# PKU-VCL-Geometry/GeoSplatting

Hardware: AMD Instinct MI355X
Metric: fwd+bwd views/sec at 2M Gaussians, 800x800 (higher is better)
Workload: dtype f32

## Files before the change

geosplatting_amd/csrc/gs_raster.hip:

```cpp
#include "gs_common.h"
#include "gs_tone.h"
#include <stdlib.h>

#pragma clang fp contract(off)

#define GS_TILE 16
#define GS_ALPHA_MIN (1.0f / 255.0f)

#ifdef GS_RASTER_STATS
__device__ unsigned long long g_raster_stats[8];
extern "C" int gs_raster_stats_read(unsigned long long* host8, int reset)
{
    if (hipMemcpyFromSymbol(host8, HIP_SYMBOL(g_raster_stats), sizeof(unsigned long long) * 8) != hipSuccess) return -1;
    if (reset) { unsigned long long z[8] = {0}; if (hipMemcpyToSymbol(HIP_SYMBOL(g_raster_stats), z, sizeof(z)) != hipSuccess) return -1; }
    return 0;
}
__device__ unsigned long long g_raster_stats2[8];
extern "C" int gs_raster_stats2_read(unsigned long long* host8, int reset)
{
    if (hipMemcpyFromSymbol(host8, HIP_SYMBOL(g_raster_stats2), sizeof(unsigned long long) * 8) != hipSuccess) return -1;
    if (reset) { unsigned long long z[8] = {0}; if (hipMemcpyToSymbol(HIP_SYMBOL(g_raster_stats2), z, sizeof(z)) != hipSuccess) return -1; }
    return 0;
}
__device__ unsigned long long g_raster_stats3[8];
// ... 642 lines not shown
    int bin_final = -1;
    float v_rc[CD];
#pragma unroll
    for (int k = 0; k < CD; ++k) v_rc[k] = 0.0f;
    if (inside) {
        const size_t pid = (size_t)pyi * W + pxi;
        const float a_out = alphas[pid];
        T_final = 1.0f - a_out;
        bin_final = last_ids[pid];
        if (CD == 3 && tone.v_image) {
#pragma clang fp contract(off)
            const float e = tone.exposure[0];
            const float r = tone.render[3 * pid], gch = tone.render[3 * pid + 1], bl = tone.render[3 * pid + 2];
            const float4 g = tone.v_image[pid];
            const float gx = g.x * tone_grad(tone.mode, r * e), gy = g.y * tone_grad(tone.mode, gch * e), gz = g.z * tone_grad(tone.mode, bl * e);
            v_rc[0] = gx * e; v_rc[1] = gy * e; v_rc[2] = gz * e;
            v_a = tone.mode == GS_TONE_NONE ? g.w * e : g.w;
            v_exp = gx * r + gy * gch + gz * bl + (tone.mode == GS_TONE_NONE ? g.w * a_out : 0.0f);
        } else {
            v_a = v_alphas[pid];
#pragma unroll
            for (int k = 0; k < CD; ++k) if (k < D) v_rc[k] = v_render[pid * D + k];
        }
    }
    if (CD == 3 && tone.v_image) {
        v_exp = gs_wave_sum(v_exp);
        if (lane == 0 && v_exp != 0.0f) gs_atomic_add(tone.v_exposure, v_exp);
    }
    float bg_dot = 0.0f;
    if (background) {
#pragma unroll
        for (int k = 0; k < CD; ++k) if (k < D) bg_dot += background[k] * v_rc[k];
    }
    if (CD > 3) for (int k = 0; k < D; ++k) vrp[k * 64 + lane] = v_rc[k < CD ? k : 0];
    float T = T_final;
    float zacc = T_final * v_a - T_final * bg_dot;
    const unsigned long long lane_lt = (1ull << lane) - 1ull;

    int top = bin_final;
#pragma unroll
    for (int off = 32; off >= 1; off >>= 1) top = max(top, __shfl_xor(top, off, 64));
    if (top >= end) top = end - 1;

    int qhead = 0, qcount = 0;
    top = __builtin_amdgcn_readfirstlane(top);
    RawBatch raw0, raw1, raw2;
    raw_load(raw0, rec0, rec1, rec2, top - lane, top - lane >= start);
    raw_load(raw1, rec0, rec1, rec2, top - 64 - lane, top - 64 - lane >= start);
    raw_load(raw2, rec0, rec1, rec2, top - 128 - lane, top - 128 - lane >= start);
    int phase = 0;
    for (;;) {
        { GS_PHASE_BEGIN();
#define BWD_FILL_STEP(B)                                                                                               \
        {                                                                                                              \
            const unsigned long long act_b = __ballot(bin_final >= top - 63);                                          \
            int n_hit = 0;                                                                                             \
            raw_wait(B);                                                                                               \
            if (act_b != 0ull) {                                                                                       \
                float rcx, rcy, rex, rey;                                                                              \
                active_rect_c(act_b, qx0, qy0, rcx, rcy, rex, rey);                                                    \
                GS_STAT(4, 1);                                                                                         \
                n_hit = lanes_cull_append(q, B, top - lane >= start, top - lane, lane, rcx, rcy, rex, rey, qhead + qcount); \
            }                                                                                                          \
            raw_load(B, rec0, rec1, rec2, top - 192 - lane, top - 192 - lane >= start);                                \
            qcount += n_hit;                                                                                           \
            top -= 64;                                                                                                 \
        }
        LANES_FILL(qcount < 64 && top >= start, BWD_FILL_STEP)
#undef BWD_FILL_STEP
        GS_PHASE_END(0); }
        if (qcount == 0) break;
        int nb = qcount < 64 ? qcount : 64;
        lanes_lds_sync();
        GS_PHASE_BEGIN();
        const int idx_low = q.idx[(qhead + nb - 1) & (GS_LANES_Q - 1)];
        const bool live = bin_final >= idx_low;
        const unsigned long long act = __ballot(live);
        const int myslot = (qhead + lane) & (GS_LANES_Q - 1);
        const float4 ra4 = q.a[myslot];
        const float2 rb4 = q.b[myslot];
        unsigned long long pm = 0ull;
        if (act != 0ull) {
            int xmin, xmax, ymin, ymax;
            active_rect_i(act, xmin, xmax, ymin, ymax);
            pm = record_pixel_mask(lane < nb, ra4.x, ra4.y, ra4.z, ra4.w, rb4.x, rb4.y, qx0, qy0, xmin, xmax, ymin, ymax) & act;
        }
        const int cnt = __popcll(pm);
        int cum = cnt;
        cum = gs_wave_incl_scan(cum);
        if (__ballot(cum > GS_PAIR_CAP) != 0ull) {
            nb = min(nb, __popcll(__ballot(cum <= GS_PAIR_CAP)));
            if (lane >= nb) pm = 0ull;
        }
        msk[lane] = pm;
        pbase[lane] = cum - cnt;
        if (CD > 3) {
            const float* cg = colors + (size_t)__float_as_int(q.c[myslot].w) * D;
            for (int k = 0; k < D; ++k) colp[k * 64 + lane] = lane < nb ? cg[k] : 0.0f;
        }
        unsigned long long list = gs_bit_transpose64(pm, lane);
        GS_STAT(5, nb);
#ifdef GS_RASTER_STATS
        GS_STAT2(1, 1);
        GS_STAT2_ALL(0, __popcll(list));
        { int _mx = __popcll(list);
          for (int _o = 32; _o >= 1; _o >>= 1) _mx = max(_mx, __shfl_xor(_mx, _o, 64));
          GS_STAT2(6, _mx); }
#endif
        lanes_lds_sync();
        GS_PHASE_END(1);
        long long _pw0 = 0;
#ifdef GS_RASTER_PHASES
        if (blockIdx.x == 0 && threadIdx.x == 0) { _pw0 = (long long)__builtin_readcyclecounter(); atomicAdd(&g_raster_stats[6], 1ull); }
#endif
        while (__ballot(list != 0ull) != 0ull) {
            GS_STAT(6, 1);
#ifdef GS_RASTER_PHASES
            if (blockIdx.x == 0 && threadIdx.x == 0) atomicAdd(&g_raster_stats[5], 1ull);
#endif
            const bool has0 = list != 0ull;
            const int j0 = gs_pop_lowest(list);
            const bool has1 = list != 0ull;
            const int j1 = gs_pop_lowest(list);
            const int slot0 = (qhead + j0) & (GS_LANES_Q - 1), slot1 = (qhead + j1) & (GS_LANES_Q - 1);
            const float4 a0 = q.a[slot0], a1 = q.a[slot1];
            const float2 b0 = q.b[slot0], b1 = q.b[slot1];
            const float4 c0 = q.c[slot0], c1 = q.c[slot1];
            const int idx0 = q.idx[slot0], idx1 = q.idx[slot1];
            const int e0 = pbase[j0] + __popcll(msk[j0] & lane_lt), e1 = pbase[j1] + __popcll(msk[j1] & lane_lt);
            v2f sigma, ov, alpha, ra;
            {
#pragma clang fp contract(off)
                const v2f d0 = v2f{a0.x, a0.y} - pxy, d1 = v2f{a1.x, a1.y} - pxy;
                const v2f p0 = v2f{a0.z, a0.w} * v2f{d0.x, d0.x}, p1 = v2f{a1.z, a1.w} * v2f{d1.x, d1.x};
                sigma.x = gs_sigma_xy(d0, p0, b0.x);
                sigma.y = gs_sigma_xy(d1, p1, b1.x);
                ov = v2f{b0.y, b1.y} * gs_exp_neg_live2(sigma);
                alpha = __builtin_elementwise_min(ov, (v2f)(0.999f));
                ra = gs_rcp_exact2((v2f)(1.0f) - alpha);
            }
            const bool ok0 = has0 && idx0 <= bin_final && sigma.x >= 0.0f && alpha.x >= GS_ALPHA_MIN;
            const bool ok1 = has1 && idx1 <= bin_final && sigma.y >= 0.0f && alpha.y >= GS_ALPHA_MIN;
            {
                const float Tn = T * ra.x;
                const float fac = ok0 ? alpha.x * Tn : 0.0f;
                float cv;
                if (CD <= 3) {
                    cv = c0.x * v_rc[0];
                    if (CD > 1) cv = fmaf(c0.y, v_rc[1], cv);
                    if (CD > 2) cv = fmaf(c0.z, v_rc[2], cv);
                } else {
                    cv = 0.0f;
#pragma unroll
                    for (int k = 0; k < CD; ++k) if (k < D) cv = fmaf(colp[k * 64 + j0], v_rc[k], cv);
                }
                const float v_alpha = fmaf(Tn, cv, ra.x * zacc);
                const float s_out = (ok0 && ov.x <= 0.999f) ? -ov.x * v_alpha : 0.0f;
                zacc = fmaf(-fac, cv, zacc);
                T = ok0 ? Tn : T;
#ifdef GS_RASTER_STATS
                if (ok0) GS_STAT_ALL(7, 1);
                if (has0 && !ok0) { if (idx0 > bin_final) GS_STAT2_ALL(2, 1); else GS_STAT2_ALL(3, 1); }
#endif
                if (has0) pairbuf[e0] = make_float2(s_out, fac);
            }
            {
                const float Tn = T * ra.y;
                const float fac = ok1 ? alpha.y * Tn : 0.0f;
                float cv;
                if (CD <= 3) {
                    cv = c1.x * v_rc[0];
                    if (CD > 1) cv = fmaf(c1.y, v_rc[1], cv);
                    if (CD > 2) cv = fmaf(c1.z, v_rc[2], cv);
                } else {
                    cv = 0.0f;
#pragma unroll
                    for (int k = 0; k < CD; ++k) if (k < D) cv = fmaf(colp[k * 64 + j1], v_rc[k], cv);
                }
                const float v_alpha = fmaf(Tn, cv, ra.y * zacc);
                const float s_out = (ok1 && ov.y <= 0.999f) ? -ov.y * v_alpha : 0.0f;
                zacc = fmaf(-fac, cv, zacc);
                T = ok1 ? Tn : T;
#ifdef GS_RASTER_STATS
                if (ok1) GS_STAT_ALL(7, 1);
                if (has1 && !ok1) { if (idx1 > bin_final) GS_STAT2_ALL(2, 1); else GS_STAT2_ALL(3, 1); }
#endif
                if (has1) pairbuf[e1] = make_float2(s_out, fac);
            }
        }
        lanes_lds_sync();
#ifdef GS_RASTER_PHASES
        if (blockIdx.x == 0 && threadIdx.x == 0) { const long long _t = (long long)__builtin_readcyclecounter(); atomicAdd(&g_raster_stats[2], (unsigned long long)(_t - _pw0)); _pw0 = _t; }
#endif
        float sum[NV];
        {
            const float X = ra4.x - ((float)qx0 + 0.5f), Y = ra4.y - ((float)qy0 + 0.5f);
            unsigned long long m = pm;
            int e = cum - cnt;
            float m0 = 0.0f, mxy = 0.0f, c2 = 0.0f;
            v2f m1 = (v2f)(0.0f), m2 = (v2f)(0.0f), c01 = (v2f)(0.0f);
            float csum[CD > 3 ? CD : 1];
#pragma unroll
            for (int k = 0; k < (CD > 3 ? CD : 1); ++k) csum[k] = 0.0f;
            while (__ballot(m != 0ull) != 0ull) {
                GS_STAT2(7, 1);
#ifdef GS_RASTER_PHASES
                if (blockIdx.x == 0 && threadIdx.x == 0) atomicAdd(&g_raster_stats[7], 1ull);
#endif
                const bool has = m != 0ull;
                const int p = gs_pop_lowest(m);
                const float2 sfr = pairbuf[has ? e : 0];
                float4 vr = make_float4(0.f, 0.f, 0.f, 0.f);
                if (CD <= 3) { vr.x = __shfl(v_rc[0], p, 64); vr.y = CD > 1 ? __shfl(v_rc[1], p, 64) : 0.0f; vr.z = CD > 2 ? __shfl(v_rc[2], p, 64) : 0.0f; }
                if (CD > 3) {
                    const float fw = has ? sfr.y : 0.0f;
#pragma unroll
                    for (int k = 0; k < CD; ++k) if (k < D) csum[k] = fmaf(fw, vrp[k * 64 + p], csum[k]);
                }
                e += has ? 1 : 0;
                const float s_w = has ? sfr.x : 0.0f, f_w = has ? sfr.y : 0.0f;
                const v2f d = v2f{X, Y} - v2f{(float)(p & 7), (float)(p >> 3)};
                const v2f sd = d * s_w;
                m0 += s_w;
                m1 += sd;
                m2 = __builtin_elementwise_fma(sd, d, m2);
                mxy = fmaf(sd.x, d.y, mxy);
                c01 = __builtin_elementwise_fma((v2f)(f_w), v2f{vr.x, vr.y}, c01);
                if (CD > 2) c2 = fmaf(f_w, vr.z, c2);
            }
            sum[0] = m0; sum[1] = m1.x; sum[2] = m1.y; sum[3] = m2.x; sum[4] = mxy; sum[5] = m2.y;
            if (CD <= 3) {
                sum[6] = c01.x;
                if (CD > 1) sum[7] = c01.y;
                if (CD > 2) sum[8] = c2;
            } else {
#pragma unroll
                for (int k = 0; k < CD; ++k) sum[6 + k] = csum[k];
            }
        }
        lanes_lds_sync();
#ifdef GS_RASTER_PHASES
        if (blockIdx.x == 0 && threadIdx.x == 0) { const long long _t = (long long)__builtin_readcyclecounter(); atomicAdd(&g_raster_stats[3], (unsigned long long)(_t - _pw0)); _pw0 = _t; }
#endif
        {
            const float ga = ra4.z, gb = ra4.w, gc = rb4.x, go = rb4.y;
            const float M0 = sum[0], Mx = sum[1], My = sum[2];
            float out[NV];
            out[0] = (2.0f * ga) * Mx + gb * My;
            out[1] = gb * Mx + (2.0f * gc) * My;
            out[2] = 0.5f * sum[3]; out[3] = sum[4]; out[4] = 0.5f * sum[5];
            out[5] = (M0 != 0.0f) ? -M0 / go : 0.0f;
#pragma unroll
            for (int k = 0; k < CD; ++k) out[6 + k] = sum[6 + k];
            if (lane < nb) {
#pragma unroll
                for (int k = 0; k < NV; ++k) stage[lane * NV + k] = out[k];
            }
        }
        lanes_lds_sync();
        {
            const int r = lane / NV, k = lane - r * NV;
            for (int it = 0; it * RPI < nb; ++it) {
                const int j = it * RPI + r;
                if (r < RPI && j < nb && k < 6 + D) {
                    const float v = stage[j * NV + k];
                    if (v != 0.0f) {
                        const int g = __float_as_int(q.c[(qhead + j) & (GS_LANES_Q - 1)].w);
                        gs_atomic_add(v_packed + (size_t)g * rec_stride + k, v);
                    }
                }
            }
        }
        lanes_lds_sync();
#ifdef GS_RASTER_PHASES
        if (blockIdx.x == 0 && threadIdx.x == 0) atomicAdd(&g_raster_stats[4], (unsigned long long)((long long)__builtin_readcyclecounter() - _pw0));
#endif
        qhead = (qhead + nb) & (GS_LANES_Q - 1);
        qcount -= nb;
    }
    raw_drain(raw0, raw1, raw2);
    GS_TL_END();
}

static constexpr int GS_LOG_PAIR_CAP = 790;
#ifndef GS_LOG_ASSIST_MAX
#define GS_LOG_ASSIST_MAX 16
#endif
static_assert(GS_LOG_ASSIST_MAX >= 0 && GS_LOG_ASSIST_MAX <= 64, "an assisted trip serves at most the 64 pixels of one wave");
struct LogLds {
    static constexpr int Q_BYTES = 64 * (16 + 16 + 8 + 4);
    static constexpr int OFF_MSK = Q_BYTES;
    static constexpr int OFF_BASE = OFF_MSK + 64 * 8;
    static constexpr int OFF_PAIR = OFF_BASE + 64 * 4;
    static constexpr int OFF_APIX = OFF_PAIR + (GS_LOG_PAIR_CAP + 2) * 8;
    static constexpr int WAVE_BYTES = OFF_APIX + (GS_LOG_ASSIST_MAX > 16 ? GS_LOG_ASSIST_MAX : 16) * 4;
};

template <int CTRL>
__device__ __forceinline__ float gs_row_shr(float ident, float src)
{
    return __builtin_bit_cast(float, __builtin_amdgcn_update_dpp(__builtin_bit_cast(int, ident), __builtin_bit_cast(int, src), CTRL, 0xf, 0xf, false));
}

template <int CD>
__global__ void __launch_bounds__(256)
raster_bwd_log_kernel(int W, int H, int tile_w, int n_tiles, int D, const int32_t* __restrict__ tile_order,
                      const float4* __restrict__ rec0, const float4* __restrict__ rec1, const float4* __restrict__ rec2,
                      const float* __restrict__ background, GsCount ic, const int32_t* __restrict__ offsets,
                      const float* __restrict__ alphas, const int32_t* __restrict__ last_ids,
                      const float* __restrict__ v_render, const float* __restrict__ v_alphas,
                      float* __restrict__ v_packed, int rec_stride, ToneBwd tone, CullLog log, BwdOrder bo)
{
    const int n_isects = (int)gs_count(ic);
#if defined(GS_RASTER_STATS) && !defined(GS_RASTER_PHASES)
    int walk_hist[8] = { 0, 0, 0, 0, 0, 0, 0, 0 };
#endif
    static_assert(CD <= 3, "colours come from the record stream (D <= 3)");
    using LD = LogLds;
    constexpr int NV = 6 + CD;
    constexpr int RPI = 64 / NV;
    static_assert(64 * NV * 4 <= GS_LOG_PAIR_CAP * 8, "the commit staging aliases the pair buffer");
    extern __shared__ __align__(16) unsigned char gs_lds_raw[];
    const int lane = threadIdx.x & 63, wave = __builtin_amdgcn_readfirstlane((int)(threadIdx.x >> 6));
    int tile;
    if (bo.bcount) {
        const int c = bo.bcount[lane];
        int incl = c;
        incl = gs_wave_incl_scan(incl);
        const unsigned long long above = __ballot(incl > (int)blockIdx.x);
        const int b = above ? __builtin_ctzll(above) : 63;
        const int before = __builtin_amdgcn_readlane(incl - c, b);
        tile = __builtin_amdgcn_readlane(incl, 63) == n_tiles
                   ? __builtin_amdgcn_readfirstlane(bo.blist[(size_t)b * n_tiles + ((int)blockIdx.x - before)]) : tile_order[blockIdx.x];
    } else {
        tile = tile_order[blockIdx.x];
    }
    const int tx = tile % tile_w, ty = tile / tile_w;
    const int qx0 = tx * GS_TILE + (wave & 1) * 8, qy0 = ty * GS_TILE + (wave >> 1) * 8;
    const int pxi = qx0 + (lane & 7), pyi = qy0 + (lane >> 3);
    const bool inside = pxi < W && pyi < H;
    const float px = (float)pxi + 0.5f, py = (float)pyi + 0.5f;
    const v2f pxy = v2f{px, py};

    const int start = offsets[tile];
    const int end = (tile == n_tiles - 1) ? n_isects : offsets[tile + 1];
    GS_TL_BEGIN(end - start);
    if (end <= start) { GS_TL_END(); return; }

    unsigned char* wbase = gs_lds_raw + (size_t)wave * LD::WAVE_BYTES;
    float4* qa = (float4*)wbase; float4* qc = qa + 64; float2* qb = (float2*)(qc + 64); int* qidx = (int*)(qb + 64);
    unsigned long long* msk = (unsigned long long*)(wbase + LD::OFF_MSK);
    int* pbase = (int*)(wbase + LD::OFF_BASE);
    float2* pairbuf = (float2*)(wbase + LD::OFF_PAIR);
    int* apix = (int*)(wbase + LD::OFF_APIX);
    float* stage = (float*)(wbase + LD::OFF_PAIR);

    float T_final = 1.0f, v_a = 0.0f, v_exp = 0.0f;
    int bin_final = -1;
    float v_rc[CD];
#pragma unroll
    for (int k = 0; k < CD; ++k) v_rc[k] = 0.0f;
    if (inside) {
        const size_t pid = (size_t)pyi * W + pxi;
        const float a_out = alphas[pid];
        T_final = 1.0f - a_out;
        bin_final = last_ids[pid];
        if (CD == 3 && tone.v_image) {
#pragma clang fp contract(off)
            const float e = tone.exposure[0];
            const float r = tone.render[3 * pid], gch = tone.render[3 * pid + 1], bl = tone.render[3 * pid + 2];
            const float4 g = tone.v_image[pid];
            const float gx = g.x * tone_grad(tone.mode, r * e), gy = g.y * tone_grad(tone.mode, gch * e), gz = g.z * tone_grad(tone.mode, bl * e);
            v_rc[0] = gx * e; v_rc[1] = gy * e; v_rc[2] = gz * e;
            v_a = tone.mode == GS_TONE_NONE ? g.w * e : g.w;
            v_exp = gx * r + gy * gch + gz * bl + (tone.mode == GS_TONE_NONE ? g.w * a_out : 0.0f);
        } else {
            v_a = v_alphas[pid];
#pragma unroll
            for (int k = 0; k < CD; ++k) if (k < D) v_rc[k] = v_render[pid * D + k];
        }
    }
    if (CD == 3 && tone.v_image) {
        v_exp = gs_wave_sum(v_exp);
        if (lane == 0 && v_exp != 0.0f) gs_atomic_add(tone.v_exposure, v_exp);
    }
    float bg_dot = 0.0f;
    if (background) {
#pragma unroll
        for (int k = 0; k < CD; ++k) if (k < D) bg_dot += background[k] * v_rc[k];
    }
    float T = T_final;
    float zacc = T_final * v_a - T_final * bg_dot;
    const unsigned long long lane_lt = (1ull << lane) - 1ull;

    int pos = __builtin_amdgcn_readfirstlane(log.count[4 * tile + wave]);
    if (pos <= 0) { GS_TL_END(); return; }
    const size_t log_base = 4 * (size_t)start + (size_t)wave * (size_t)(end - start);
    const int32_t* lidx = log.idx + log_base;
    const unsigned long long* lmsk = log.mask + log_base;
    int e_idx, g_idx; unsigned long long e_msk, g_msk;
    float4 g0, g1, g2;
    {
        const int e = pos - 1 - lane;
        const int es = e >= 0 ? e : 0;
        g_idx = lidx[es]; g_msk = e >= 0 ? lmsk[es] : 0ull;
        g0 = rec0[g_idx]; g1 = rec1[g_idx]; g2 = rec2[g_idx];
        const int e2 = pos - 65 - lane;
        const int es2 = e2 >= 0 ? e2 : 0;
        e_idx = lidx[es2]; e_msk = e2 >= 0 ? lmsk[es2] : 0ull;
    }
    while (pos > 0) {
        const int nb = pos < 64 ? pos : 64;
        const float4 c0 = g0, c1 = g1, c2 = g2;
        const int c_idx = g_idx;
        const unsigned long long c_msk = g_msk;
        g_idx = e_idx; g_msk = e_msk;
        g0 = rec0[g_idx]; g1 = rec1[g_idx]; g2 = rec2[g_idx];
        {
            const int e2 = pos - 129 - lane;
            const int es2 = e2 >= 0 ? e2 : 0;
            e_idx = lidx[es2]; e_msk = e2 >= 0 ? lmsk[es2] : 0ull;
        }
        pos -= nb;
        GS_PHASE_BEGIN();
        lanes_lds_sync();
        qa[lane] = c0; qb[lane] = make_float2(c1.x, c1.y); qc[lane] = c2; qidx[lane] = c_idx;
        GS_STAT(5, nb);
        const int idx_low = __builtin_amdgcn_readlane(c_idx, nb - 1);
        const bool live = bin_final >= idx_low;
        const unsigned long long act = __ballot(live);
        const unsigned long long pm = lane < nb ? (c_msk & act) : 0ull;
        if (__ballot(pm != 0ull) == 0ull) { GS_PHASE_END(1); continue; }
        const float4 ra4 = c0;
        const float2 rb4 = make_float2(c1.x, c1.y);
        const int cnt = __popcll(pm);
        int cum = cnt;
        cum = gs_wave_incl_scan(cum);
        GS_PHASE_END(1);
        int r0 = 0, cumbase = 0;
        while (r0 < nb) {
            const int r1 = r0 + __popcll(__ballot(lane >= r0 && lane < nb && (cum - cumbase) <= GS_LOG_PAIR_CAP));
            const bool mine = lane >= r0 && lane < r1;
            const unsigned long long pms = mine ? pm : 0ull;
            lanes_lds_sync();
            msk[lane] = pms;
            pbase[lane] = cum - cnt - cumbase;
            unsigned long long list = gs_bit_transpose64(pms, lane);
#ifdef GS_RASTER_STATS
            GS_STAT2(1, 1);
            GS_STAT2_ALL(0, __popcll(list));
#endif
            lanes_lds_sync();
            long long _pw0 = 0;
#ifdef GS_RASTER_PHASES
            if (blockIdx.x == 0 && threadIdx.x == 0) { _pw0 = (long long)__builtin_readcyclecounter(); atomicAdd(&g_raster_stats[6], 1ull); }
#endif
            if (__ballot(list != 0ull) != 0ull) do {
                GS_STAT(6, 1);
#if defined(GS_RASTER_STATS) && !defined(GS_RASTER_PHASES)
                { const int na = __popcll(__ballot(list != 0ull));
#pragma unroll
                  for (int k = 0; k < 8; ++k) walk_hist[k] += (na > 8 * k && na <= 8 * k + 8) ? 1 : 0; }
#endif
#ifdef GS_RASTER_PHASES
                if (blockIdx.x == 0 && threadIdx.x == 0) atomicAdd(&g_raster_stats[5], 1ull);
#endif
#if GS_LOG_ASSIST_MAX > 0
                {
                    const unsigned long long am = __ballot(list != 0ull);
                    const int na = __popcll(am);
                    if (na <= GS_LOG_ASSIST_MAX && __ballot(__popcll(list) > 2) != 0ull) {
                        const int gs = na <= 8 ? 3 : (GS_LOG_ASSIST_MAX <= 16 || na <= 16) ? 2 : na <= 32 ? 1 : 0, G = 1 << gs;
                        const int rank = __popcll(am & lane_lt);
                        lanes_lds_sync();
                        if (list != 0ull) apix[rank] = lane;
                        lanes_lds_sync();
                        const int g = lane >> gs, h = lane & (G - 1);
                        const bool grp = g < na;
                        const int p = grp ? apix[g] : 0;
                        const int pa = p << 2;
                        unsigned long long L = ((unsigned long long)(unsigned)__builtin_amdgcn_ds_bpermute(pa, (int)(unsigned)(list >> 32)) << 32) |
                                               (unsigned long long)(unsigned)__builtin_amdgcn_ds_bpermute(pa, (int)(unsigned)list);
                        const float T0 = __builtin_bit_cast(float, __builtin_amdgcn_ds_bpermute(pa, __builtin_bit_cast(int, T)));
                        const float Z0 = __builtin_bit_cast(float, __builtin_amdgcn_ds_bpermute(pa, __builtin_bit_cast(int, zacc)));
                        const int bf = __builtin_amdgcn_ds_bpermute(pa, bin_final);
                        float vr[CD];
#pragma unroll
                        for (int c = 0; c < CD; ++c) vr[c] = __builtin_bit_cast(float, __builtin_amdgcn_ds_bpermute(pa, __builtin_bit_cast(int, v_rc[c])));
                        if (!grp) L = 0ull;
                        for (int i = 0; i < G - 1; ++i) L = (i < h) ? (L & (L - 1ull)) : L;
                        const bool has = L != 0ull;
                        const int j = gs_pop_lowest(L);
                        const float4 a = qa[j]; const float2 b = qb[j]; const float4 cc = qc[j];
                        const int idx = qidx[j];
                        const unsigned long long below = (1ull << p) - 1ull;
                        const int e = pbase[j] + __popcll(msk[j] & below);
                        float sigma, ov, alpha, ra;
                        {
#pragma clang fp contract(off)
                            const v2f d = v2f{a.x, a.y} - v2f{(float)(qx0 + (p & 7)) + 0.5f, (float)(qy0 + (p >> 3)) + 0.5f};
                            const v2f pp = v2f{a.z, a.w} * v2f{d.x, d.x};
                            sigma = gs_sigma_xy(d, pp, b.x);
                            ov = b.y * __builtin_amdgcn_exp2f(sigma * -1.4426950408889634f);
                            alpha = fminf(ov, 0.999f);
                            const float x = 1.0f - alpha;
                            const float r0 = __builtin_amdgcn_rcpf(x);
                            ra = fmaf(r0, fmaf(-x, r0, 1.0f), r0);
                        }
                        const bool ok = has & (idx <= bf) & (sigma >= 0.0f) & (alpha >= GS_ALPHA_MIN);
                        float cv = cc.x * vr[0];
                        if (CD > 1) cv = fmaf(cc.y, vr[1], cv);
                        if (CD > 2) cv = fmaf(cc.z, vr[2], cv);
                        float pi = ok ? ra : 1.0f;
                        { const float t = gs_row_shr<0x111>(1.0f, pi); pi *= (h >= 1) ? t : 1.0f; }
                        { const float t = gs_row_shr<0x112>(1.0f, pi); pi *= (h >= 2) ? t : 1.0f; }
                        { const float t = gs_row_shr<0x114>(1.0f, pi); pi *= (h >= 4) ? t : 1.0f; }
                        float pe = gs_row_shr<0x111>(1.0f, pi); pe = (h >= 1) ? pe : 1.0f;
                        const float Tb = T0 * pe, Tn = Tb * ra;
                        const float fac = ok ? alpha * Tn : 0.0f;
                        float si = fac * cv;
                        { const float t = gs_row_shr<0x111>(0.0f, si); si += (h >= 1) ? t : 0.0f; }
                        { const float t = gs_row_shr<0x112>(0.0f, si); si += (h >= 2) ? t : 0.0f; }
                        { const float t = gs_row_shr<0x114>(0.0f, si); si += (h >= 4) ? t : 0.0f; }
                        float se = gs_row_shr<0x111>(0.0f, si); se = (h >= 1) ? se : 0.0f;
                        const float zb = Z0 - se;
                        const float v_alpha = fmaf(Tn, cv, ra * zb);
                        const float s_out = (ok && ov <= 0.999f) ? -ov * v_alpha : 0.0f;
#ifdef GS_RASTER_STATS
                        if (ok) GS_STAT_ALL(7, 1);
                        if (has && !ok) { if (idx > bf) GS_STAT2_ALL(2, 1); else GS_STAT2_ALL(3, 1); }
#endif
                        pairbuf[has ? e : GS_LOG_PAIR_CAP] = make_float2(s_out, fac);
                        const float T_end = T0 * pi, Z_end = Z0 - si;
                        const int src = (((rank << gs) + G - 1) & 63) << 2;
                        const float Tg = __builtin_bit_cast(float, __builtin_amdgcn_ds_bpermute(src, __builtin_bit_cast(int, T_end)));
                        const float Zg = __builtin_bit_cast(float, __builtin_amdgcn_ds_bpermute(src, __builtin_bit_cast(int, Z_end)));
                        const unsigned Llo = (unsigned)__builtin_amdgcn_ds_bpermute(src, (int)(unsigned)L);
                        const unsigned Lhi = (unsigned)__builtin_amdgcn_ds_bpermute(src, (int)(unsigned)(L >> 32));
                        if (list != 0ull) { T = Tg; zacc = Zg; list = ((unsigned long long)Lhi << 32) | Llo; }
                        continue;
                    }
                }
#endif
                const bool has0 = list != 0ull;
                const int j0 = gs_pop_lowest(list);
                const bool has1 = list != 0ull;
                const int j1 = gs_pop_lowest(list);
                const float4 a0 = qa[j0], a1 = qa[j1];
                const float2 b0 = qb[j0], b1 = qb[j1];
                const float4 cc0 = qc[j0], cc1 = qc[j1];
                const int idx0 = qidx[j0], idx1 = qidx[j1];
                const int e0 = pbase[j0] + __popcll(msk[j0] & lane_lt), e1 = pbase[j1] + __popcll(msk[j1] & lane_lt);
                v2f sigma, ov, alpha, ra;
                {
#pragma clang fp contract(off)
                    const v2f d0 = v2f{a0.x, a0.y} - pxy, d1 = v2f{a1.x, a1.y} - pxy;
                    const v2f p0 = v2f{a0.z, a0.w} * v2f{d0.x, d0.x}, p1 = v2f{a1.z, a1.w} * v2f{d1.x, d1.x};
                    sigma.x = gs_sigma_xy(d0, p0, b0.x);
                    sigma.y = gs_sigma_xy(d1, p1, b1.x);
#ifndef GS_BWD_LOG_EXACT_MATH
                    ov = v2f{b0.y, b1.y} * v2f{__builtin_amdgcn_exp2f(sigma.x * -1.4426950408889634f), __builtin_amdgcn_exp2f(sigma.y * -1.4426950408889634f)};
                    alpha = __builtin_elementwise_min(ov, (v2f)(0.999f));
                    {
                        const v2f x = (v2f)(1.0f) - alpha;
                        const v2f r0 = v2f{__builtin_amdgcn_rcpf(x.x), __builtin_amdgcn_rcpf(x.y)};
                        ra = __builtin_elementwise_fma(r0, __builtin_elementwise_fma(-x, r0, (v2f)(1.0f)), r0);
                    }
#else
                    ov = v2f{b0.y, b1.y} * gs_exp_neg_live2(sigma);
                    alpha = __builtin_elementwise_min(ov, (v2f)(0.999f));
                    ra = gs_rcp_exact2((v2f)(1.0f) - alpha);
#endif
                }
                const bool ok0 = has0 & (idx0 <= bin_final) & (sigma.x >= 0.0f) & (alpha.x >= GS_ALPHA_MIN);
                const bool ok1 = has1 & (idx1 <= bin_final) & (sigma.y >= 0.0f) & (alpha.y >= GS_ALPHA_MIN);
                {
                    const float Tn = T * ra.x;
                    const float fac = ok0 ? alpha.x * Tn : 0.0f;
                    float cv = cc0.x * v_rc[0];
                    if (CD > 1) cv = fmaf(cc0.y, v_rc[1], cv);
                    if (CD > 2) cv = fmaf(cc0.z, v_rc[2], cv);
                    const float v_alpha = fmaf(Tn, cv, ra.x * zacc);
                    const float s_out = (ok0 && ov.x <= 0.999f) ? -ov.x * v_alpha : 0.0f;
                    zacc = fmaf(-fac, cv, zacc);
                    T = ok0 ? Tn : T;
#ifdef GS_RASTER_STATS
                    if (ok0) GS_STAT_ALL(7, 1);
                    if (has0 && !ok0) { if (idx0 > bin_final) GS_STAT2_ALL(2, 1); else GS_STAT2_ALL(3, 1); }
#endif
                    pairbuf[has0 ? e0 : GS_LOG_PAIR_CAP] = make_float2(s_out, fac);
                }
                {
                    const float Tn = T * ra.y;
                    const float fac = ok1 ? alpha.y * Tn : 0.0f;
                    float cv = cc1.x * v_rc[0];
                    if (CD > 1) cv = fmaf(cc1.y, v_rc[1], cv);
                    if (CD > 2) cv = fmaf(cc1.z, v_rc[2], cv);
                    const float v_alpha = fmaf(Tn, cv, ra.y * zacc);
                    const float s_out = (ok1 && ov.y <= 0.999f) ? -ov.y * v_alpha : 0.0f;
                    zacc = fmaf(-fac, cv, zacc);
                    T = ok1 ? Tn : T;
#ifdef GS_RASTER_STATS
                    if (ok1) GS_STAT_ALL(7, 1);
                    if (has1 && !ok1) { if (idx1 > bin_final) GS_STAT2_ALL(2, 1); else GS_STAT2_ALL(3, 1); }
#endif
                    pairbuf[has1 ? e1 : GS_LOG_PAIR_CAP] = make_float2(s_out, fac);
                }
            } while (__ballot(list != 0ull) != 0ull);
            lanes_lds_sync();
#ifdef GS_RASTER_PHASES
            if (blockIdx.x == 0 && threadIdx.x == 0) { const long long _t = (long long)__builtin_readcyclecounter(); atomicAdd(&g_raster_stats[2], (unsigned long long)(_t - _pw0)); _pw0 = _t; }
#endif
            float sum[NV];
            {
                const float X = ra4.x - ((float)qx0 + 0.5f), Y = ra4.y - ((float)qy0 + 0.5f);
                unsigned long long m = pms;
                int e = cum - cnt - cumbase;
                float m0 = 0.0f, mxy = 0.0f, c2s = 0.0f;
                v2f m1 = (v2f)(0.0f), m2 = (v2f)(0.0f), c01 = (v2f)(0.0f);
                if (__ballot(m != 0ull) != 0ull) do {
                    GS_STAT2(7, 1);
#ifdef GS_RASTER_PHASES
                    if (blockIdx.x == 0 && threadIdx.x == 0) atomicAdd(&g_raster_stats[7], 1ull);
#endif
                    const bool has = m != 0ull;
                    const int p = gs_pop_lowest(m);
                    const float2 sfr = pairbuf[has ? e : 0];
                    float4 vr;
                    vr.x = __shfl(v_rc[0], p, 64); vr.y = CD > 1 ? __shfl(v_rc[1], p, 64) : 0.0f; vr.z = CD > 2 ? __shfl(v_rc[2], p, 64) : 0.0f; vr.w = 0.0f;
                    e += has ? 1 : 0;
                    const float s_w = has ? sfr.x : 0.0f, f_w = has ? sfr.y : 0.0f;
                    const v2f d = v2f{X, Y} - v2f{(float)(p & 7), (float)(p >> 3)};
                    const v2f sd = d * s_w;
                    m0 += s_w;
                    m1 += sd;
                    m2 = __builtin_elementwise_fma(sd, d, m2);
                    mxy = fmaf(sd.x, d.y, mxy);
                    c01 = __builtin_elementwise_fma((v2f)(f_w), v2f{vr.x, vr.y}, c01);
                    if (CD > 2) c2s = fmaf(f_w, vr.z, c2s);
                } while (__ballot(m != 0ull) != 0ull);
                sum[0] = m0; sum[1] = m1.x; sum[2] = m1.y; sum[3] = m2.x; sum[4] = mxy; sum[5] = m2.y;
                sum[6] = c01.x;
                if (CD > 1) sum[7] = c01.y;
                if (CD > 2) sum[8] = c2s;
            }
            lanes_lds_sync();
#ifdef GS_RASTER_PHASES
            if (blockIdx.x == 0 && threadIdx.x == 0) { const long long _t = (long long)__builtin_readcyclecounter(); atomicAdd(&g_raster_stats[3], (unsigned long long)(_t - _pw0)); _pw0 = _t; }
#endif
            {
                const float ga = ra4.z, gb = ra4.w, gc = rb4.x, go = rb4.y;
                const float M0 = sum[0], Mx = sum[1], My = sum[2];
                float out[NV];
                out[0] = (2.0f * ga) * Mx + gb * My;
                out[1] = gb * Mx + (2.0f * gc) * My;
                out[2] = 0.5f * sum[3]; out[3] = sum[4]; out[4] = 0.5f * sum[5];
                out[5] = (M0 != 0.0f) ? -M0 / go : 0.0f;
#pragma unroll
                for (int k = 0; k < CD; ++k) out[6 + k] = sum[6 + k];
                if (mine) {
#pragma unroll
                    for (int k = 0; k < NV; ++k) stage[lane * NV + k] = out[k];
                }
            }
            lanes_lds_sync();
            {
                const int r = lane / NV, k = lane - r * NV;
                for (int it = 0; r0 + it * RPI < r1; ++it) {
                    const int j = r0 + it * RPI + r;
                    if (r < RPI && j < r1 && k < 6 + D) {
                        const float v = stage[j * NV + k];
                        if (v != 0.0f) {
                            const int g = __float_as_int(qc[j].w);
                            gs_atomic_add(v_packed + (size_t)g * rec_stride + k, v);
                        }
                    }
                }
            }
#ifdef GS_RASTER_PHASES
            if (blockIdx.x == 0 && threadIdx.x == 0) atomicAdd(&g_raster_stats[4], (unsigned long long)((long long)__builtin_readcyclecounter() - _pw0));
#endif
            cumbase = __builtin_amdgcn_readlane(cum, r1 - 1);
            r0 = r1;
        }
    }
#if defined(GS_RASTER_STATS) && !defined(GS_RASTER_PHASES)
    if (lane == 0) {
#pragma unroll
        for (int k = 0; k < 8; ++k) if (walk_hist[k]) atomicAdd(&g_raster_stats3[k], (unsigned long long)walk_hist[k]);
    }
#endif
    GS_TL_END();
}

#define GS_RASTER_BLOCKS_PER_CU 4
static int gs_raster_blocks_per_cu() { return GS_RASTER_BLOCKS_PER_CU; }
static size_t gs_raster_lds_pad() { return (size_t)(160 * 1024 / gs_raster_blocks_per_cu()) - 1024; }
static size_t gs_raster_lds(size_t natural)
{
    const size_t pad = gs_raster_lds_pad();
    if (natural >= pad) return natural;
    if ((size_t)(gs_raster_blocks_per_cu() + 1) * (natural + 512) > (size_t)160 * 1024) return natural;
    return pad;
}
static size_t align256(size_t x) { return (x + 255) & ~(size_t)255; }

extern "C" size_t gs_raster_ws_bytes(int64_t n_isects, int V, int W, int H, int tile_size)
{
    if (tile_size <= 0) return 0;
    const size_t tiles = (size_t)((W + tile_size - 1) / tile_size) * (size_t)((H + tile_size - 1) / tile_size);
    const size_t n = n_isects > 0 ? (size_t)n_isects : 1;
    const size_t v = V > 0 ? (size_t)V : 1;
    return 3 * align256(n * sizeof(float4)) + align256(tiles * sizeof(int32_t)) + align256(64 * sizeof(int32_t)) +
           align256(64 * tiles * sizeof(int32_t)) + align256(4 * v * sizeof(float4));
}

struct RasterWs {
    float4 *rec0, *rec1, *rec2;
    int32_t* order;
    BwdOrder bo;
    float4* vis;
};
static RasterWs carve(void* ws, int64_t n_isects, int V, int tiles)
{
    const size_t n = n_isects > 0 ? (size_t)n_isects : 1;
    const size_t v = V > 0 ? (size_t)V : 1;
    char* p = (char*)ws;
    RasterWs r;
    r.rec0 = (float4*)p; p += align256(n * sizeof(float4));
    r.rec1 = (float4*)p; p += align256(n * sizeof(float4));
    r.rec2 = (float4*)p; p += align256(n * sizeof(float4));
    r.order = (int32_t*)p; p += align256((size_t)tiles * sizeof(int32_t));
    r.bo.bcount = (int32_t*)p; p += align256(64 * sizeof(int32_t));
    r.bo.blist = (int32_t*)p; p += align256(64 * (size_t)tiles * sizeof(int32_t));
    r.vis = (float4*)p;
    return r;
}

struct RasterOpts {
    const int64_t* counts = nullptr;
    ToneFwd tone_fwd = { 0, nullptr, nullptr };
    ToneBwd tone_bwd = { 0, nullptr, nullptr, nullptr, nullptr };
    CullLog log = { nullptr, nullptr, nullptr };
};
static GsCount isect_count(int64_t n, const RasterOpts& o)
{
    return GsCount{ (long long)n, o.counts ? (const long long*)o.counts + 1 : nullptr };
}

template <int CD>
static int launch_fwd(int W, int H, int D, const RasterWs& ws, const float* colors, const float* background,
                      int64_t n_isects, const int32_t* offsets, float* render, float* alphas, int32_t* last_ids,
                      hipStream_t s, const RasterOpts& o)
{
    const int tile_w = (W + GS_TILE - 1) / GS_TILE, tile_h = (H + GS_TILE - 1) / GS_TILE;
    if (o.tone_fwd.image && !(CD == 3 && D == 3 && background == nullptr)) {
        gs_set_error("gs_raster_composite_tone: needs D == 3 and no background");
        return GS_EINVAL;
    }
    {
        const size_t planes = CD > 3 ? 4 * (size_t)2 * (size_t)D * 64 * sizeof(float) : 0;
        const size_t lds = gs_raster_lds(4 * (size_t)GS_WIN_Q_BYTES + planes);
        if (lds > 64 * 1024)
            GS_CHECK_HIP(hipFuncSetAttribute((const void*)raster_fwd_window_kernel<CD>, hipFuncAttributeMaxDynamicSharedMemorySize, (int)lds));
        hipLaunchKernelGGL(raster_fwd_window_kernel<CD>, dim3(tile_w * tile_h), dim3(256), lds, s, W, H, tile_w, tile_w * tile_h, D,
                           ws.order, ws.rec0, ws.rec1, ws.rec2, colors, background, isect_count(n_isects, o), offsets, render, alphas,
                           last_ids, o.tone_fwd, o.log, o.log.count ? ws.bo : BwdOrder{ nullptr, nullptr });
        GS_CHECK_LAUNCH();
        return GS_OK;
    }
}

static int raster_check(const char* who, int W, int H, int tile_size, int D, int V, int64_t n_isects, const void* ws,
                        size_t ws_bytes)
{
    GS_CHECK_ARG(W > 0 && H > 0, "bad image size");
    GS_CHECK_ARG(tile_size == GS_TILE, "only tile_size=16 is built (rfstudio/model/gsplat.py:30)");
    GS_CHECK_ARG(D >= 1 && D <= GS_MAX_CHANNELS, "1 <= D <= 32");
    GS_CHECK_ARG(n_isects >= 0 && n_isects < (1ll << 31), "n_isects must fit int32");
    GS_CHECK_ARG(ws != nullptr, "workspace must not be NULL");
    GS_CHECK_ARG(V >= 0, "bad V");
    if (ws_bytes < gs_raster_ws_bytes(n_isects, V, W, H, tile_size)) { gs_set_error("%s: workspace too small", who); return GS_ENOSPC; }
    return GS_OK;
}

static int raster_prepare_impl(int W, int H, int tile_size, int D, int V, const float* means2d, const float* conics,
                               const float* opacities, const float* colors, const float* vis_records, int64_t n_isects,
                               const int32_t* offsets, const int32_t* flatten_ids, void* ws, size_t ws_bytes, void* stream,
                               const RasterOpts& o)
{
    const int rc = raster_check("gs_raster_prepare", W, H, tile_size, D, V, n_isects, ws, ws_bytes);
    if (rc != GS_OK) return rc;
    hipStream_t s = (hipStream_t)stream;
    const int tiles = ((W + GS_TILE - 1) / GS_TILE) * ((H + GS_TILE - 1) / GS_TILE);
    const RasterWs r = carve(ws, n_isects, V, tiles);
    if (n_isects > 0 && V > 0) {
        const float4* vis = (const float4*)vis_records;
        if (!vis) {
            hipLaunchKernelGGL(pack_visible_kernel, dim3(gs_cdiv(V, 256)), dim3(256), 0, s, V, D, means2d, conics, opacities, colors,
                               r.vis);
            GS_CHECK_LAUNCH();
            vis = r.vis;
        }
        hipLaunchKernelGGL(build_stream_packed_kernel, dim3(gs_cdiv(n_isects, 256)), dim3(256), 0, s, isect_count(n_isects, o), flatten_ids,
                           vis, r.rec0, r.rec1, r.rec2);
        GS_CHECK_LAUNCH();
    }
    hipLaunchKernelGGL(tile_order_kernel, dim3(1), dim3(1024), 0, s, tiles, isect_count(n_isects, o), offsets, r.order, r.bo);
    GS_CHECK_LAUNCH();
    return GS_OK;
}

static int raster_composite_impl(int W, int H, int tile_size, int D, int V, const float* colors, const float* background,
                                 int64_t n_isects, const int32_t* offsets, float* render, float* alphas, int32_t* last_ids,
                                 const void* ws, size_t ws_bytes, void* stream, const RasterOpts& o)
{
    const int rc = raster_check("gs_raster_composite", W, H, tile_size, D, V, n_isects, ws, ws_bytes);
    if (rc != GS_OK) return rc;
    hipStream_t s = (hipStream_t)stream;
    const int tiles = ((W + GS_TILE - 1) / GS_TILE) * ((H + GS_TILE - 1) / GS_TILE);
    const RasterWs r = carve((void*)ws, n_isects, V, tiles);
#define GS_FWD(CD) return launch_fwd<CD>(W, H, D, r, colors, background, n_isects, offsets, render, alphas, last_ids, s, o)
    if (D <= 3) GS_FWD(3);
    if (D <= 4) GS_FWD(4);
    if (D <= 8) GS_FWD(8);
    if (D <= 16) GS_FWD(16);
    GS_FWD(32);
#undef GS_FWD
}

template <int CD>
static int launch_bwd(int W, int H, int D, const RasterWs& ws, const float* colors, const float* background,
                      int64_t n_isects, const int32_t* offsets, const float* alphas, const int32_t* last_ids,
                      const float* v_render, const float* v_alphas, float* v_packed, int rec_stride, hipStream_t s,
                      const RasterOpts& o)
{
    const int tile_w = (W + GS_TILE - 1) / GS_TILE, tile_h = (H + GS_TILE - 1) / GS_TILE;
    if (o.tone_bwd.v_image && !(CD == 3 && D == 3 && background == nullptr)) {
        gs_set_error("gs_raster_bwd_tone: needs D == 3 and no background");
        return GS_EINVAL;
    }
    if constexpr (CD <= 3) {
        if (o.log.idx) {
            const size_t lds = gs_raster_lds(4 * (size_t)LogLds::WAVE_BYTES);
            hipLaunchKernelGGL(raster_bwd_log_kernel<CD>, dim3(tile_w * tile_h), dim3(256), lds, s, W, H, tile_w, tile_w * tile_h, D,
                               ws.order, ws.rec0, ws.rec1, ws.rec2, background, isect_count(n_isects, o), offsets, alphas, last_ids,
                               v_render, v_alphas, v_packed, rec_stride, o.tone_bwd, o.log, ws.bo);
            GS_CHECK_LAUNCH();
            return GS_OK;
        }
    }
    {
        size_t lds = 4 * ((size_t)Lanes2Lds<CD>::WAVE_BYTES + (CD > 3 ? 2 * (size_t)D * 64 * 4 : 0));
        if (lds < gs_raster_lds_pad()) lds = gs_raster_lds_pad();
        if (lds > 64 * 1024)
            GS_CHECK_HIP(hipFuncSetAttribute((const void*)raster_bwd_lanes2_kernel<CD>, hipFuncAttributeMaxDynamicSharedMemorySize, (int)lds));
        hipLaunchKernelGGL(raster_bwd_lanes2_kernel<CD>, dim3(tile_w * tile_h), dim3(256), lds, s, W, H, tile_w, tile_w * tile_h, D,
                           ws.order, ws.rec0, ws.rec1, ws.rec2, colors, background, isect_count(n_isects, o), offsets, alphas, last_ids,
                           v_render, v_alphas, v_packed, rec_stride, o.tone_bwd);
        GS_CHECK_LAUNCH();
        return GS_OK;
    }
}

extern "C" int gs_raster_grad_stride(int D) { return ((6 + D) + 15) / 16 * 16; }

static int raster_bwd_impl(int W, int H, int tile_size, int D, int V, const float* colors, const float* background,
                           int64_t n_isects, const int32_t* offsets, const float* alphas, const int32_t* last_ids,
                           const float* v_render, const float* v_alphas, float* v_packed, const void* ws,
                           size_t ws_bytes, void* stream, bool zero, const RasterOpts& o)
{
    const int rc = raster_check("gs_raster_bwd", W, H, tile_size, D, V, n_isects, ws, ws_bytes);
    if (rc != GS_OK) return rc;
    hipStream_t s = (hipStream_t)stream;
    const int rec_stride = gs_raster_grad_stride(D);
    if (V > 0 && zero) GS_CHECK_HIP(gs_zero_async(v_packed, sizeof(float) * (size_t)rec_stride * (size_t)V, s));
    if (n_isects == 0 || V == 0) return GS_OK;
    const int tiles = ((W + GS_TILE - 1) / GS_TILE) * ((H + GS_TILE - 1) / GS_TILE);
    const RasterWs r = carve((void*)ws, n_isects, V, tiles);
#define GS_BWD(CD) return launch_bwd<CD>(W, H, D, r, colors, background, n_isects, offsets, alphas, last_ids, v_render, v_alphas, v_packed, rec_stride, s, o)
    if (D <= 3) GS_BWD(3);
    if (D <= 4) GS_BWD(4);
    if (D <= 8) GS_BWD(8);
    if (D <= 16) GS_BWD(16);
    GS_BWD(32);
#undef GS_BWD
}

static CullLog carve_log(const void* log_ws, int64_t n_isects)
{
    const size_t n = n_isects > 0 ? (size_t)n_isects : 1;
    char* p = (char*)log_ws;
    CullLog l;
    l.mask = (unsigned long long*)p; p += align256(4 * n * sizeof(unsigned long long));
    l.idx = (int32_t*)p; p += align256(4 * n * sizeof(int32_t));
    l.count = (int32_t*)p;
    return l;
}
extern "C" size_t gs_raster_log_ws_bytes(int64_t n_isects, int W, int H, int tile_size)
{
    if (tile_size <= 0) return 0;
    const size_t n = n_isects > 0 ? (size_t)n_isects : 1;
    const size_t tiles = (size_t)((W + tile_size - 1) / tile_size) * (size_t)((H + tile_size - 1) / tile_size);
    return align256(4 * n * sizeof(unsigned long long)) + align256(4 * n * sizeof(int32_t)) + align256(4 * tiles * sizeof(int32_t));
}

extern "C" int gs_raster_prepare(int W, int H, int tile_size, int D, int V, const float* means2d, const float* conics,
                                 const float* opacities, const float* colors, int64_t n_isects, const int32_t* offsets,
                                 const int32_t* flatten_ids, void* ws, size_t ws_bytes, void* stream)
{
    return raster_prepare_impl(W, H, tile_size, D, V, means2d, conics, opacities, colors, nullptr, n_isects, offsets, flatten_ids,
                               ws, ws_bytes, stream, RasterOpts{});
}

extern "C" int gs_raster_prepare_vis(int W, int H, int tile_size, int D, int V, const float* vis_records, int64_t n_isects,
                                     const int32_t* offsets, const int32_t* flatten_ids, void* ws, size_t ws_bytes, void* stream)
{
    GS_CHECK_ARG(vis_records != nullptr || V == 0, "vis_records (written by gs_project_fwd_vis) must not be NULL");
    return raster_prepare_impl(W, H, tile_size, D, V, nullptr, nullptr, nullptr, nullptr, vis_records, n_isects, offsets,
                               flatten_ids, ws, ws_bytes, stream, RasterOpts{});
}

extern "C" int gs_raster_composite(int W, int H, int tile_size, int D, int V, const float* colors, const float* background,
                                   int64_t n_isects, const int32_t* offsets, float* render, float* alphas,
                                   int32_t* last_ids, const void* ws, size_t ws_bytes, void* stream)
{
    return raster_composite_impl(W, H, tile_size, D, V, colors, background, n_isects, offsets, render, alphas, last_ids, ws,
                                 ws_bytes, stream, RasterOpts{});
}

extern "C" int gs_raster_fwd(int W, int H, int tile_size, int D, int V, const float* means2d, const float* conics,
                             const float* opacities, const float* colors, const float* background,
                             int64_t n_isects, const int32_t* offsets, const int32_t* flatten_ids,
                             float* render, float* alphas, int32_t* last_ids, void* ws, size_t ws_bytes, void* stream)
{
    const int rc = raster_prepare_impl(W, H, tile_size, D, V, means2d, conics, opacities, colors, nullptr, n_isects, offsets,
                                       flatten_ids, ws, ws_bytes, stream, RasterOpts{});
    if (rc != GS_OK) return rc;
    return raster_composite_impl(W, H, tile_size, D, V, colors, background, n_isects, offsets, render, alphas, last_ids, ws,
                                 ws_bytes, stream, RasterOpts{});
}

extern "C" int gs_raster_bwd(int W, int H, int tile_size, int D, int V, const float* colors, const float* background,
                             int64_t n_isects, const int32_t* offsets, const float* alphas, const int32_t* last_ids,
                             const float* v_render, const float* v_alphas, float* v_packed, const void* ws,
                             size_t ws_bytes, void* stream)
{
    return raster_bwd_impl(W, H, tile_size, D, V, colors, background, n_isects, offsets, alphas, last_ids, v_render, v_alphas,
                           v_packed, ws, ws_bytes, stream, true, RasterOpts{});
}

extern "C" int gs_raster_bwd_acc(int W, int H, int tile_size, int D, int V, const float* colors, const float* background,
                                 int64_t n_isects, const int32_t* offsets, const float* alphas, const int32_t* last_ids,
                                 const float* v_render, const float* v_alphas, float* v_packed, const void* ws,
                                 size_t ws_bytes, void* stream)
{
    return raster_bwd_impl(W, H, tile_size, D, V, colors, background, n_isects, offsets, alphas, last_ids, v_render, v_alphas,
                           v_packed, ws, ws_bytes, stream, false, RasterOpts{});
}

extern "C" int gs_raster_prepare_vis_cap(int W, int H, int tile_size, int D, int V_cap, const float* vis_records, int64_t n_isects_cap,
                                         const int64_t* counts_dev, const int32_t* offsets, const int32_t* flatten_ids, void* ws,
                                         size_t ws_bytes, void* stream)
{
    GS_CHECK_ARG(counts_dev != nullptr, "counts_dev must not be NULL");
    GS_CHECK_ARG(vis_records != nullptr || V_cap == 0, "vis_records (written by gs_project_fwd_vis) must not be NULL");
    RasterOpts o;
    o.counts = counts_dev;
    return raster_prepare_impl(W, H, tile_size, D, V_cap, nullptr, nullptr, nullptr, nullptr, vis_records, n_isects_cap, offsets,
                               flatten_ids, ws, ws_bytes, stream, o);
}

extern "C" int gs_raster_composite_cap(int W, int H, int tile_size, int D, int V_cap, const float* colors, const float* background,
                                       int64_t n_isects_cap, const int64_t* counts_dev, const int32_t* offsets, float* render,
                                       float* alphas, int32_t* last_ids, const void* ws, size_t ws_bytes, void* stream)
{
    GS_CHECK_ARG(counts_dev != nullptr, "counts_dev must not be NULL");
    RasterOpts o;
    o.counts = counts_dev;
// ... 140 lines not shown
```

Baseline: 768.6.

## Prefetch next log batch with inline-asm loads and pair atomic commits

Replaces compiler-scheduled prefetch of the next batch's Gaussian records and log entries with inline-asm global loads, so they stay in flight across the whole batch and are only waited on just before the atomic commit. The record load for rec1 shrinks to a dwordx2. The atomic commit loop is unrolled by two, with clamped indices, so two LDS reads and two atomics are issued per iteration. The cost is manual vmcnt(0) waits that also drain other outstanding loads, held registers, and fragile inline asm.

Result: faster. 777.4 (median of 6 runs) (+1.1%).

```diff
diff --git a/geosplatting_amd/csrc/gs_raster.hip b/geosplatting_amd/csrc/gs_raster.hip
--- a/geosplatting_amd/csrc/gs_raster.hip
+++ b/geosplatting_amd/csrc/gs_raster.hip
@@ -968,6 +968,25 @@
     return __builtin_bit_cast(float, __builtin_amdgcn_update_dpp(__builtin_bit_cast(int, ident), __builtin_bit_cast(int, src), CTRL, 0xf, 0xf, false));
 }
 
+struct LogPrefetch { v4f r0; v2f r1; v4f r2; int e_idx; unsigned long long e_msk; };
+__device__ __forceinline__ void log_load(LogPrefetch& p, const float4* p0, const float4* p1, const float4* p2, const int32_t* pi,
+                                         const unsigned long long* pm)
+{
+    asm volatile("global_load_dwordx4 %0, %1, off" : "=&v"(p.r0) : "v"(p0) : "memory");
+    asm volatile("global_load_dwordx2 %0, %1, off" : "=&v"(p.r1) : "v"(p1) : "memory");
+    asm volatile("global_load_dwordx4 %0, %1, off" : "=&v"(p.r2) : "v"(p2) : "memory");
+    asm volatile("global_load_dword %0, %1, off" : "=&v"(p.e_idx) : "v"(pi) : "memory");
+    asm volatile("global_load_dwordx2 %0, %1, off" : "=&v"(p.e_msk) : "v"(pm) : "memory");
+}
+__device__ __forceinline__ void log_wait(LogPrefetch& p)
+{
+    asm volatile("s_waitcnt vmcnt(0)" : : "v"(p.r0), "v"(p.r1), "v"(p.r2), "v"(p.e_idx), "v"(p.e_msk) : "memory");
+}
+__device__ __forceinline__ void log_take(LogPrefetch& p)
+{
+    asm volatile("" : "+v"(p.r0), "+v"(p.r1), "+v"(p.r2), "+v"(p.e_idx), "+v"(p.e_msk) : : "memory");
+}
+
 template <int CD>
 __global__ void __launch_bounds__(256)
 raster_bwd_log_kernel(int W, int H, int tile_w, int n_tiles, int D, const int32_t* __restrict__ tile_order,
@@ -1064,41 +1083,45 @@
     const size_t log_base = 4 * (size_t)start + (size_t)wave * (size_t)(end - start);
     const int32_t* lidx = log.idx + log_base;
     const unsigned long long* lmsk = log.mask + log_base;
-    int e_idx, g_idx; unsigned long long e_msk, g_msk;
-    float4 g0, g1, g2;
+    int g_idx; unsigned long long g_msk;
+    LogPrefetch pf;
+    bool e_ok;
     {
         const int e = pos - 1 - lane;
         const int es = e >= 0 ? e : 0;
         g_idx = lidx[es]; g_msk = e >= 0 ? lmsk[es] : 0ull;
-        g0 = rec0[g_idx]; g1 = rec1[g_idx]; g2 = rec2[g_idx];
         const int e2 = pos - 65 - lane;
         const int es2 = e2 >= 0 ? e2 : 0;
-        e_idx = lidx[es2]; e_msk = e2 >= 0 ? lmsk[es2] : 0ull;
+        e_ok = e2 >= 0;
+        log_load(pf, rec0 + g_idx, rec1 + g_idx, rec2 + g_idx, lidx + es2, lmsk + es2);
+        log_wait(pf);
     }
     while (pos > 0) {
         const int nb = pos < 64 ? pos : 64;
-        const float4 c0 = g0, c1 = g1, c2 = g2;
+        log_take(pf);
+        const float4 c0 = make_float4(pf.r0.x, pf.r0.y, pf.r0.z, pf.r0.w), c2 = make_float4(pf.r2.x, pf.r2.y, pf.r2.z, pf.r2.w);
+        const float2 c1 = make_float2(pf.r1.x, pf.r1.y);
         const int c_idx = g_idx;
         const unsigned long long c_msk = g_msk;
-        g_idx = e_idx; g_msk = e_msk;
-        g0 = rec0[g_idx]; g1 = rec1[g_idx]; g2 = rec2[g_idx];
+        g_idx = pf.e_idx; g_msk = e_ok ? pf.e_msk : 0ull;
         {
             const int e2 = pos - 129 - lane;
             const int es2 = e2 >= 0 ? e2 : 0;
-            e_idx = lidx[es2]; e_msk = e2 >= 0 ? lmsk[es2] : 0ull;
+            e_ok = e2 >= 0;
+            log_load(pf, rec0 + g_idx, rec1 + g_idx, rec2 + g_idx, lidx + es2, lmsk + es2);
         }
         pos -= nb;
         GS_PHASE_BEGIN();
         lanes_lds_sync();
-        qa[lane] = c0; qb[lane] = make_float2(c1.x, c1.y); qc[lane] = c2; qidx[lane] = c_idx;
+        qa[lane] = c0; qb[lane] = c1; qc[lane] = c2; qidx[lane] = c_idx;
         GS_STAT(5, nb);
         const int idx_low = __builtin_amdgcn_readlane(c_idx, nb - 1);
         const bool live = bin_final >= idx_low;
         const unsigned long long act = __ballot(live);
         const unsigned long long pm = lane < nb ? (c_msk & act) : 0ull;
-        if (__ballot(pm != 0ull) == 0ull) { GS_PHASE_END(1); continue; }
+        if (__ballot(pm != 0ull) == 0ull) { GS_PHASE_END(1); log_wait(pf); continue; }
         const float4 ra4 = c0;
-        const float2 rb4 = make_float2(c1.x, c1.y);
+        const float2 rb4 = c1;
         const int cnt = __popcll(pm);
         int cum = cnt;
         cum = gs_wave_incl_scan(cum);
@@ -1330,17 +1353,18 @@
                 }
             }
             lanes_lds_sync();
+            log_wait(pf);
             {
                 const int r = lane / NV, k = lane - r * NV;
-                for (int it = 0; r0 + it * RPI < r1; ++it) {
-                    const int j = r0 + it * RPI + r;
-                    if (r < RPI && j < r1 && k < 6 + D) {
-                        const float v = stage[j * NV + k];
-                        if (v != 0.0f) {
-                            const int g = __float_as_int(qc[j].w);
-                            gs_atomic_add(v_packed + (size_t)g * rec_stride + k, v);
-                        }
-                    }
+                const bool lane_ok = r < RPI && k < 6 + D;
+                for (int ja = r0 + r; ja - r < r1; ja += 2 * RPI) {
+                    const int jb = ja + RPI;
+                    const int jca = ja < r1 ? ja : r1 - 1, jcb = jb < r1 ? jb : r1 - 1;
+                    const float va = stage[jca * NV + k], vb = stage[jcb * NV + k];
+                    int ga = __float_as_int(qc[jca].w), gb = __float_as_int(qc[jcb].w);
+                    asm volatile("" : "+v"(ga), "+v"(gb));
+                    if (lane_ok && ja < r1 && va != 0.0f) gs_atomic_add(v_packed + (size_t)ga * rec_stride + k, va);
+                    if (lane_ok && jb < r1 && vb != 0.0f) gs_atomic_add(v_packed + (size_t)gb * rec_stride + k, vb);
                 }
             }
 #ifdef GS_RASTER_PHASES
```
